# eridgd/WCT-TF

Hardware: AMD Instinct MI355X
Metric: stylized frames/sec @512x512, 5-level relu5->1 pipeline, alpha=0.8 (higher is better)
Workload: dtype f16

## Files before the change

### wct_tf_amd/csrc/conv_wino.hip

```cpp
#include "common.h"

namespace {
typedef unsigned int u32x4 __attribute__((ext_vector_type(4)));
typedef _Float16 h2 __attribute__((ext_vector_type(2)));
constexpr int TW = 16;
constexpr int PITCH = 20;
constexpr int BK = 32;

__device__ __forceinline__ half8 pk_sub(half8 a, half8 b) {
  u32x4 ua = __builtin_bit_cast(u32x4, a), ub = __builtin_bit_cast(u32x4, b), r;
#pragma unroll
  for (int i = 0; i < 4; ++i) {
    unsigned o;
    asm("v_pk_add_f16 %0, %1, %2 neg_lo:[0,1] neg_hi:[0,1]" : "=v"(o) : "v"(ua[i]), "v"(ub[i]));
    r[i] = o;
  }
  return __builtin_bit_cast(half8, r);
}

__device__ __forceinline__ int reflect_idx(int i, int n) {
  if (i < 0) i = -i;
  if (i >= n) i = 2 * n - 2 - i;
  i = i < 0 ? 0 : i;
  return i >= n ? n - 1 : i;
}

template <int TH, int BN, int WM, int WN, bool IL>
__global__ __launch_bounds__(256, TH >= 16 ? 1 : 2)
void conv3x3_wino_kernel(ConvArgs p, int tiles_x, int n_tiles) {
  constexpr int PR = TH / 2;
  constexpr int MT = (PR / 2) / WM;
  constexpr int NT = (BN / 32) / WN;
  constexpr int G = 256 / PR;
  constexpr int SL = (72 + G - 1) / G;
  constexpr int PATCH_BYTES = PR * 4 * PITCH * 64;
  constexpr int DUMP_OFF = 2 * PATCH_BYTES;
  constexpr int PF_TAP = 5;
  static_assert(PR % 2 == 0 && (PR / 2) % WM == 0 && 256 % PR == 0 && WM * WN == 4, "tile shape");

  extern __shared__ __attribute__((aligned(16))) unsigned char smem[];
  const int tid = threadIdx.x, lane = tid & 63, wave = tid >> 6;
  const int wm = wave / WN, wn = wave % WN;
  int bid = blockIdx.x;
  const int ntile = bid % n_tiles;
  bid /= n_tiles;
  const int tx = bid % tiles_x, ty = bid / tiles_x;
  const int b = blockIdx.y;
  const int y0 = ty * TH, x0 = tx * TW, n0 = ntile * BN;

  const int Hin = p.upsample ? p.H / 2 : p.H;
  const int Win = p.upsample ? p.W / 2 : p.W;
  const half_t* xb = p.x + (size_t)b * Hin * Win * p.Cin;
  const __amdgpu_buffer_rsrc_t w_rsrc = __builtin_amdgcn_make_buffer_rsrc((void*)p.w_wino, 0, 0x7FFFFFFF, 0x00020000);
  const __amdgpu_buffer_rsrc_t x_rsrc = __builtin_amdgcn_make_buffer_rsrc((void*)xb, 0, 0x7FFFFFFF, 0x00020000);

  const int lpr = tid / G, ls = tid % G;
  unsigned row_off[4], col_off[SL], dst_off[SL];
  bool slot_ok[SL];
#pragma unroll
  for (int i = 0; i < 4; ++i) {
    int iy = reflect_idx(y0 + 2 * lpr - 1 + i, p.H);
    if (p.upsample) iy >>= 1;
    row_off[i] = (unsigned)(iy * Win) * p.Cin * 2;
  }
#pragma unroll
  for (int j = 0; j < SL; ++j) {
    const int slot = ls + j * G;
    slot_ok[j] = slot < 72;
    const int px = slot_ok[j] ? slot >> 2 : 0, piece = slot & 3;
    int ix = reflect_idx(x0 - 1 + px, p.W);
    if (p.upsample) ix >>= 1;
    col_off[j] = (unsigned)(ix * p.Cin + piece * 8) * 2;
    dst_off[j] = ((lpr * 4 * PITCH + px) * 4 + (piece ^ ((px >> 2) & 3))) * 16;
    if (IL && !slot_ok[j]) dst_off[j] = DUMP_OFF + tid * 16;
  }
  u32x4 raw[SL][4];
  auto load_rows = [&](int chunk) {
#pragma unroll
    for (int j = 0; j < SL; ++j)
#pragma unroll
      for (int i = 0; i < 4; ++i)
        raw[j][i] = __builtin_amdgcn_raw_buffer_load_b128(x_rsrc, row_off[i] + col_off[j], chunk * BK * 2, 0);
  };
  auto park_rows = [&](int buf) {
#pragma unroll
    for (int j = 0; j < SL; ++j) {
      const half8 d0 = __builtin_bit_cast(half8, raw[j][0]), d1 = __builtin_bit_cast(half8, raw[j][1]);
      const half8 d2 = __builtin_bit_cast(half8, raw[j][2]), d3 = __builtin_bit_cast(half8, raw[j][3]);
      const half8 t0 = pk_sub(d0, d2), t1 = d1 + d2, t2 = pk_sub(d2, d1), t3 = pk_sub(d1, d3);
      if (slot_ok[j]) {
        unsigned char* d = smem + buf * PATCH_BYTES + dst_off[j];
        *reinterpret_cast<half8*>(d) = t0;
        *reinterpret_cast<half8*>(d + PITCH * 64) = t1;
        *reinterpret_cast<half8*>(d + 2 * PITCH * 64) = t2;
        *reinterpret_cast<half8*>(d + 3 * PITCH * 64) = t3;
      }
    }
  };

  const int frag_px = lane & 15, frag_pr = (lane & 31) >> 4, kgrp = lane >> 5;
  int rd_base[3][2];
#pragma unroll
  for (int kx = 0; kx < 3; ++kx)
#pragma unroll
    for (int ks = 0; ks < 2; ++ks) {
      const int px = frag_px + kx;
      rd_base[kx][ks] = (((wm * MT * 2 + frag_pr) * 4) * PITCH + px) * 64 + (((ks * 2 + kgrp) ^ ((px >> 2) & 3)) * 16);
    }
  const int c16 = p.Cin >> 4;
  unsigned wfrag[NT];
#pragma unroll
  for (int nt = 0; nt < NT; ++nt) wfrag[nt] = (((n0 >> 5) + wn * NT + nt) * 12 * c16 * 512 + lane * 8) * 2;

  f32x16 acc[4][NT][MT];
#pragma unroll
  for (int nt = 0; nt < NT; ++nt) {
    f32x4 bv[4];
#pragma unroll
    for (int rq = 0; rq < 4; ++rq) bv[rq] = *reinterpret_cast<const f32x4*>(p.bias + n0 + (wn * NT + nt) * 32 + 8 * rq + 4 * kgrp);
#pragma unroll
    for (int f = 0; f < 4; ++f)
#pragma unroll
      for (int mt = 0; mt < MT; ++mt)
#pragma unroll
        for (int r = 0; r < 16; ++r) acc[f][nt][mt][r] = f == 1 ? bv[r >> 2][r & 3] : 0.f;
  }

  const int n_chunks = p.Cin / BK;
  half8 wf[3][NT][2];
  half8 bf[IL ? 3 : 2][2][MT];
  auto load_w = [&](half8 (&dst)[NT][2], int tap12, int chunk) {
    const int soff = (tap12 * c16 + chunk * 2) * 1024;
#pragma unroll
    for (int nt = 0; nt < NT; ++nt)
#pragma unroll
      for (int ks = 0; ks < 2; ++ks)
        dst[nt][ks] = __builtin_bit_cast(half8, __builtin_amdgcn_raw_buffer_load_b128(w_rsrc, wfrag[nt] + ks * 1024, soff, 0));
  };
  auto read_b = [&](half8 (&dst)[2][MT], int f, int kx, int buf) {
#pragma unroll
    for (int ks = 0; ks < 2; ++ks)
#pragma unroll
      for (int mt = 0; mt < MT; ++mt)
        dst[ks][mt] = *reinterpret_cast<const half8*>(smem + buf * PATCH_BYTES + rd_base[kx][ks] + (mt * 8 + f) * PITCH * 64);
  };

  if constexpr (IL) {
    constexpr int NM = 2 * MT * NT;
    constexpr int NR = 2 * NT + 2 * MT;
#ifndef WINO_LT0
#define WINO_LT0 1
#define WINO_PT0 6
#endif
    constexpr int LT0 = WINO_LT0, PT0 = WINO_PT0;
    static_assert(LT0 + SL <= PT0 && PT0 + SL <= 10, "staging schedule");
#ifndef WINO_WRING
#define WINO_WRING 4
#endif
#ifndef WINO_ABL
#define WINO_ABL 0
#endif
#ifndef WINO_RAW_AUX
#define WINO_RAW_AUX 0
#endif
    constexpr int ABL = WINO_ABL;
    constexpr int WR = WINO_WRING, WA = WR - 1;
    static_assert(24 % WR == 0, "ring");
    half8 wq[WR][NT][2];
    half8 tq[4];
    load_rows(0);
#pragma unroll
    for (int i = 0; i < WA; ++i) load_w(wq[i], i, 0);
#pragma unroll
    for (int j = 0; j < SL; ++j) {
      const half8 d0 = __builtin_bit_cast(half8, raw[j][0]), d1 = __builtin_bit_cast(half8, raw[j][1]);
      const half8 d2 = __builtin_bit_cast(half8, raw[j][2]), d3 = __builtin_bit_cast(half8, raw[j][3]);
      unsigned char* d = smem + dst_off[j];
      *reinterpret_cast<half8*>(d) = pk_sub(d0, d2);
      *reinterpret_cast<half8*>(d + PITCH * 64) = d1 + d2;
      *reinterpret_cast<half8*>(d + 2 * PITCH * 64) = pk_sub(d2, d1);
      *reinterpret_cast<half8*>(d + 3 * PITCH * 64) = pk_sub(d1, d3);
    }
    asm volatile("s_waitcnt lgkmcnt(0)\n\ts_barrier" ::: "memory");
    read_b(bf[0], 0, 0, 0);
    read_b(bf[1], 0, 1, 0);
#pragma unroll 1
    for (int pair = 0; pair < n_chunks; pair += 2) {
#pragma unroll
      for (int t = 0; t < 24; ++t) {
        const int tt = t % 12, chunk_i = pair + t / 12, buf = t / 12;
        const int f = tt / 3, kx = tt % 3;
        const int chunk_n = chunk_i + 1 < n_chunks ? chunk_i + 1 : chunk_i;
        const int t3 = (tt + WA) % 12, c3 = tt + WA >= 12 ? chunk_n : chunk_i;
        const int t1 = (tt + 2) % 12, buf1 = tt >= 10 ? buf ^ 1 : buf;
        const int soff3 = (t3 * c16 + c3 * 2) * 1024;
#pragma unroll
        for (int j = 0; j < NM; ++j) {
          const int ks = j / (MT * NT), mt = (j / NT) % MT, nt = j % NT;
          if (!(ABL & 4)) acc[f][nt][mt] = __builtin_amdgcn_mfma_f32_32x32x16_f16(wq[t % WR][nt][ks], bf[t % 3][ks][mt], acc[f][nt][mt], 0, 0, 0);
          else asm volatile("" :: "v"(wq[t % WR][nt][ks]), "v"(bf[t % 3][ks][mt]));
#pragma unroll
          for (int k = j * NR / NM; k < (j + 1) * NR / NM; ++k) {
            if (k < 2 * NT) {
              if (!(ABL & 1)) wq[(t + WA) % WR][k / 2][k % 2] =
                  __builtin_bit_cast(half8, __builtin_amdgcn_raw_buffer_load_b128(w_rsrc, wfrag[k / 2] + (k % 2) * 1024, soff3, 0));
            } else {
              const int kk = k - 2 * NT, ks1 = kk / MT, mt1 = kk % MT;
              if (!(ABL & 8)) bf[(t + 2) % 3][ks1][mt1] = *reinterpret_cast<const half8*>(smem + buf1 * PATCH_BYTES + rd_base[t1 % 3][ks1] + (mt1 * 8 + t1 / 3) * PITCH * 64);
            }
          }
          if (tt >= LT0 && tt < LT0 + SL) {
            const int sl = tt - LT0;
            if (j < 4 && !(ABL & 2)) raw[sl][j] = __builtin_amdgcn_raw_buffer_load_b128(x_rsrc, (ABL & 64) ? (lane & 3) * 16 + j * 64 + sl * 256 : row_off[j] + col_off[sl], (ABL & 32) ? 0 : chunk_n * BK * 2, WINO_RAW_AUX);
          }
          if (tt >= PT0 && tt < PT0 + SL && !(ABL & 16)) {
            const int sl = tt - PT0;
            {
#pragma unroll
              for (int it = j * 8 / NM; it < (j + 1) * 8 / NM; ++it) {
                const int fq = it >> 1;
                if ((it & 1) == 0) {
                  const half8 da = __builtin_bit_cast(half8, raw[sl][fq == 0 ? 0 : fq == 1 ? 1 : fq == 2 ? 2 : 1]);
                  const half8 db = __builtin_bit_cast(half8, raw[sl][fq == 0 ? 2 : fq == 1 ? 2 : fq == 2 ? 1 : 3]);
                  tq[fq] = fq == 1 ? da + db : pk_sub(da, db);
                } else {
                  *reinterpret_cast<half8*>(smem + (buf ^ 1) * PATCH_BYTES * (slot_ok[sl] ? 1 : 0) + dst_off[sl] + fq * PITCH * 64) = tq[fq];
                }
              }
            }
          }
          __builtin_amdgcn_sched_barrier(0);
        }
        if (tt == 9) asm volatile("s_waitcnt lgkmcnt(0)\n\ts_barrier" ::: "memory");
      }
    }
  } else {
  load_rows(0);
  load_w(wf[0], 0, 0);
  load_w(wf[1], 1, 0);
  park_rows(0);
  asm volatile("s_waitcnt lgkmcnt(0)\n\ts_barrier" ::: "memory");
  read_b(bf[0], 0, 0, 0);

#pragma unroll 1
  for (int pair = 0; pair < n_chunks; pair += 2) {
#pragma unroll
    for (int t = 0; t < 24; ++t) {
      const int tt = t % 12, chunk_i = pair + t / 12, buf = t / 12;
      const int f = tt / 3, kx = tt % 3;
      const bool more = chunk_i + 1 < n_chunks;
      {
        const int t2 = (tt + 2) % 12;
        const int c2 = tt + 2 >= 12 ? (more ? chunk_i + 1 : chunk_i) : chunk_i;
        load_w(wf[(t + 2) % 3], t2, c2);
      }
      if (tt == PF_TAP && more) load_rows(chunk_i + 1);
      if (tt != 11) read_b(bf[(t + 1) & 1], (tt + 1) / 3, (tt + 1) % 3, buf);
      else if (more) read_b(bf[(t + 1) & 1], 0, 0, buf ^ 1);
      __builtin_amdgcn_sched_barrier(0);
#pragma unroll
      for (int ks = 0; ks < 2; ++ks)
#pragma unroll
        for (int mt = 0; mt < MT; ++mt)
#pragma unroll
          for (int nt = 0; nt < NT; ++nt)
            acc[f][nt][mt] = __builtin_amdgcn_mfma_f32_32x32x16_f16(wf[t % 3][nt][ks], bf[t & 1][ks][mt], acc[f][nt][mt], 0, 0, 0);
      __builtin_amdgcn_sched_barrier(0);
      if (tt == 10 && more) {
        park_rows(buf ^ 1);
        asm volatile("s_waitcnt lgkmcnt(0)\n\ts_barrier" ::: "memory");
      }
    }
  }

  }
  constexpr int OOB = (int)0x80000000u;
  const int Ho = p.pool ? (p.H + 1) / 2 : p.H, Wo = p.pool ? (p.W + 1) / 2 : p.W;
  const unsigned img_elems = (unsigned)Ho * Wo * p.Cout;
  const __amdgpu_buffer_rsrc_t r16 = __builtin_amdgcn_make_buffer_rsrc((void*)(p.y16 + (size_t)b * img_elems), 0, img_elems * 2, 0x00020000);
  const float lo1 = p.relu ? 0.f : -__builtin_inff();
  const h2 lo2 = {(half_t)lo1, (half_t)lo1};
  const h2 zero2 = {(half_t)0.f, (half_t)0.f};
  const int ox = x0 + frag_px;
  const int chan = n0 + wn * NT * 32;
#pragma unroll
  for (int mt = 0; mt < MT; ++mt) {
    const int oy = y0 + ((wm * MT + mt) * 2 + frag_pr) * 2;
    const bool in0 = (oy < p.H) & (ox < p.W), in1 = (oy + 1 < p.H) & (ox < p.W);
    int off[2];
    if (p.pool) {
      off[0] = in0 && (frag_px & 1) == 0 ? (((oy >> 1) * Wo + (ox >> 1)) * p.Cout + chan + 8 * kgrp) * 2 : OOB;
      off[1] = OOB;
    } else {
      off[0] = in0 ? ((oy * p.W + ox) * p.Cout + chan + 8 * kgrp) * 2 : OOB;
      off[1] = in1 ? (((oy + 1) * p.W + ox) * p.Cout + chan + 8 * kgrp) * 2 : OOB;
    }
#pragma unroll
    for (int nt = 0; nt < NT; ++nt) {
      unsigned pk[2][4][2];
#pragma unroll
      for (int rq = 0; rq < 4; ++rq) {
        f32x4 e, o;
#pragma unroll
        for (int j = 0; j < 4; ++j) {
          const int r = rq * 4 + j;
          const float m0 = acc[0][nt][mt][r], m1 = acc[1][nt][mt][r], m2 = acc[2][nt][mt][r], m3 = acc[3][nt][mt][r];
          e[j] = (m0 + m1) + m2;
          o[j] = (m1 - m2) - m3;
        }
        h2 e0 = {(half_t)e[0], (half_t)e[1]}, e1 = {(half_t)e[2], (half_t)e[3]};
        h2 o0 = {(half_t)o[0], (half_t)o[1]}, o1 = {(half_t)o[2], (half_t)o[3]};
        e0 = __builtin_elementwise_max(e0, lo2); e1 = __builtin_elementwise_max(e1, lo2);
        o0 = __builtin_elementwise_max(o0, lo2); o1 = __builtin_elementwise_max(o1, lo2);
        if (p.pool) {
          h2 q[2] = {__builtin_elementwise_max(in0 ? e0 : zero2, in1 ? o0 : zero2), __builtin_elementwise_max(in0 ? e1 : zero2, in1 ? o1 : zero2)};
#pragma unroll
          for (int d = 0; d < 2; ++d) {
            const unsigned tq = __builtin_bit_cast(unsigned, q[d]);
            const h2 nb = __builtin_bit_cast(h2, __builtin_amdgcn_update_dpp(0, (int)tq, 0xB1, 0xF, 0xF, true));
            q[d] = __builtin_elementwise_max(q[d], nb);
          }
          e0 = q[0]; e1 = q[1];
        }
        pk[0][rq][0] = __builtin_bit_cast(unsigned, e0); pk[0][rq][1] = __builtin_bit_cast(unsigned, e1);
        pk[1][rq][0] = __builtin_bit_cast(unsigned, o0); pk[1][rq][1] = __builtin_bit_cast(unsigned, o1);
      }
#pragma unroll
      for (int par = 0; par < 2; ++par) {
#pragma unroll
        for (int m = 0; m < 2; ++m) {
          auto sx = __builtin_amdgcn_permlane32_swap(pk[par][2 * m][0], pk[par][2 * m + 1][0], false, false);
          auto sy = __builtin_amdgcn_permlane32_swap(pk[par][2 * m][1], pk[par][2 * m + 1][1], false, false);
          u32x4 ov = {sx[0], sy[0], sx[1], sy[1]};
          __builtin_amdgcn_raw_buffer_store_b128(ov, r16, off[par] + (nt * 32 + 16 * m) * 2, 0, 0);
        }
      }
    }
  }
}

template <int TH, int BN, int WM, int WN, bool IL = false>
int launch_wino_cfg(const ConvArgs& a, hipStream_t s) {
  const int tiles_x = cdiv(a.W, TW), tiles_y = cdiv(a.H, TH), n_tiles = a.Cout / BN;
  const size_t lds = 2 * (size_t)(TH / 2) * 4 * PITCH * 64 + (IL ? 8192 : 0);
  HIP_TRY(hipFuncSetAttribute(reinterpret_cast<const void*>(&conv3x3_wino_kernel<TH, BN, WM, WN, IL>),
                              hipFuncAttributeMaxDynamicSharedMemorySize, (int)lds));
  hipLaunchKernelGGL((conv3x3_wino_kernel<TH, BN, WM, WN, IL>), dim3(tiles_x * tiles_y * n_tiles, a.B), dim3(256), lds, s, a, tiles_x, n_tiles);
  HIP_TRY(hipGetLastError());
  return WCT_OK;
}
}

bool conv3x3_wino_takes(const ConvArgs& a) {
  return a.w_wino != nullptr && a.y16 != nullptr && a.y32 == nullptr && a.usum == nullptr && a.img1 == nullptr &&
         a.Cin % 64 == 0 && a.Cout % 64 == 0 && (!a.pool || a.relu);
}

int launch_conv3x3_wino(const ConvArgs& a, hipStream_t s) {
  ARG_CHECK(conv3x3_wino_takes(a) && a.H > 1 && a.W > 1 && a.B > 0);
  ARG_CHECK(!a.upsample || (a.H % 2 == 0 && a.W % 2 == 0));
  ARG_CHECK(launch_map_fits((size_t)a.H * a.W * a.Cin, 2));
  ARG_CHECK(launch_map_fits((size_t)a.H * a.W * a.Cout, 2));
  const long px16 = (long)cdiv(a.W, TW) * cdiv(a.H, 16) * a.B;
  const long px8 = (long)cdiv(a.W, TW) * cdiv(a.H, 8) * a.B;
  if (a.Cout % 128 == 0 && px16 * (a.Cout / 128) >= 256) return launch_wino_cfg<16, 128, 1, 4, true>(a, s);
  if (a.Cout % 128 == 0 && px8 * (a.Cout / 128) >= 256) return launch_wino_cfg<8, 128, 1, 4>(a, s);
  return launch_wino_cfg<8, 64, 2, 2>(a, s);
}
```

Before: 675.5.

## Make the large Winograd conv persistent, prefetching the next tile during the current one

Moves the TH=16 interleaved Winograd path into a new persistent kernel. It launches one block per CU, and each block walks the tiles with a grid stride. During the last chunk pair of a tile it stages the next tile's input rows and weights, so the prologue of each tile overlaps the previous one's compute and the launch/tail cost of many short blocks goes away. Bias is cached in LDS once per block. Risks are extra register pressure from the tile bookkeeping, and lower parallelism if a layer has few tiles or one block per CU underfills the machine.

Measured after the change: 685.3 (median of 6 runs). +1.5%, better.

```diff
diff --git a/wct_tf_amd/csrc/conv_wino.hip b/wct_tf_amd/csrc/conv_wino.hip
--- a/wct_tf_amd/csrc/conv_wino.hip
+++ b/wct_tf_amd/csrc/conv_wino.hip
@@ -25,7 +25,7 @@
   return i >= n ? n - 1 : i;
 }
 
-template <int TH, int BN, int WM, int WN, bool IL>
+template <int TH, int BN, int WM, int WN>
 __global__ __launch_bounds__(256, TH >= 16 ? 1 : 2)
 void conv3x3_wino_kernel(ConvArgs p, int tiles_x, int n_tiles) {
   constexpr int PR = TH / 2;
@@ -34,7 +34,6 @@
   constexpr int G = 256 / PR;
   constexpr int SL = (72 + G - 1) / G;
   constexpr int PATCH_BYTES = PR * 4 * PITCH * 64;
-  constexpr int DUMP_OFF = 2 * PATCH_BYTES;
   constexpr int PF_TAP = 5;
   static_assert(PR % 2 == 0 && (PR / 2) % WM == 0 && 256 % PR == 0 && WM * WN == 4, "tile shape");
 
@@ -72,7 +71,6 @@
     if (p.upsample) ix >>= 1;
     col_off[j] = (unsigned)(ix * p.Cin + piece * 8) * 2;
     dst_off[j] = ((lpr * 4 * PITCH + px) * 4 + (piece ^ ((px >> 2) & 3))) * 16;
-    if (IL && !slot_ok[j]) dst_off[j] = DUMP_OFF + tid * 16;
   }
   u32x4 raw[SL][4];
   auto load_rows = [&](int chunk) {
@@ -128,7 +126,7 @@
 
   const int n_chunks = p.Cin / BK;
   half8 wf[3][NT][2];
-  half8 bf[IL ? 3 : 2][2][MT];
+  half8 bf[2][2][MT];
   auto load_w = [&](half8 (&dst)[NT][2], int tap12, int chunk) {
     const int soff = (tap12 * c16 + chunk * 2) * 1024;
 #pragma unroll
@@ -145,15 +143,252 @@
         dst[ks][mt] = *reinterpret_cast<const half8*>(smem + buf * PATCH_BYTES + rd_base[kx][ks] + (mt * 8 + f) * PITCH * 64);
   };
 
-  if constexpr (IL) {
-    constexpr int NM = 2 * MT * NT;
-    constexpr int NR = 2 * NT + 2 * MT;
+  load_rows(0);
+  load_w(wf[0], 0, 0);
+  load_w(wf[1], 1, 0);
+  park_rows(0);
+  asm volatile("s_waitcnt lgkmcnt(0)\n\ts_barrier" ::: "memory");
+  read_b(bf[0], 0, 0, 0);
+
+#pragma unroll 1
+  for (int pair = 0; pair < n_chunks; pair += 2) {
+#pragma unroll
+    for (int t = 0; t < 24; ++t) {
+      const int tt = t % 12, chunk_i = pair + t / 12, buf = t / 12;
+      const int f = tt / 3, kx = tt % 3;
+      const bool more = chunk_i + 1 < n_chunks;
+      {
+        const int t2 = (tt + 2) % 12;
+        const int c2 = tt + 2 >= 12 ? (more ? chunk_i + 1 : chunk_i) : chunk_i;
+        load_w(wf[(t + 2) % 3], t2, c2);
+      }
+      if (tt == PF_TAP && more) load_rows(chunk_i + 1);
+      if (tt != 11) read_b(bf[(t + 1) & 1], (tt + 1) / 3, (tt + 1) % 3, buf);
+      else if (more) read_b(bf[(t + 1) & 1], 0, 0, buf ^ 1);
+      __builtin_amdgcn_sched_barrier(0);
+#pragma unroll
+      for (int ks = 0; ks < 2; ++ks)
+#pragma unroll
+        for (int mt = 0; mt < MT; ++mt)
+#pragma unroll
+          for (int nt = 0; nt < NT; ++nt)
+            acc[f][nt][mt] = __builtin_amdgcn_mfma_f32_32x32x16_f16(wf[t % 3][nt][ks], bf[t & 1][ks][mt], acc[f][nt][mt], 0, 0, 0);
+      __builtin_amdgcn_sched_barrier(0);
+      if (tt == 10 && more) {
+        park_rows(buf ^ 1);
+        asm volatile("s_waitcnt lgkmcnt(0)\n\ts_barrier" ::: "memory");
+      }
+    }
+  }
+
+  constexpr int OOB = (int)0x80000000u;
+  const int Ho = p.pool ? (p.H + 1) / 2 : p.H, Wo = p.pool ? (p.W + 1) / 2 : p.W;
+  const unsigned img_elems = (unsigned)Ho * Wo * p.Cout;
+  const __amdgpu_buffer_rsrc_t r16 = __builtin_amdgcn_make_buffer_rsrc((void*)(p.y16 + (size_t)b * img_elems), 0, img_elems * 2, 0x00020000);
+  const float lo1 = p.relu ? 0.f : -__builtin_inff();
+  const h2 lo2 = {(half_t)lo1, (half_t)lo1};
+  const h2 zero2 = {(half_t)0.f, (half_t)0.f};
+  const int ox = x0 + frag_px;
+  const int chan = n0 + wn * NT * 32;
+#pragma unroll
+  for (int mt = 0; mt < MT; ++mt) {
+    const int oy = y0 + ((wm * MT + mt) * 2 + frag_pr) * 2;
+    const bool in0 = (oy < p.H) & (ox < p.W), in1 = (oy + 1 < p.H) & (ox < p.W);
+    int off[2];
+    if (p.pool) {
+      off[0] = in0 && (frag_px & 1) == 0 ? (((oy >> 1) * Wo + (ox >> 1)) * p.Cout + chan + 8 * kgrp) * 2 : OOB;
+      off[1] = OOB;
+    } else {
+      off[0] = in0 ? ((oy * p.W + ox) * p.Cout + chan + 8 * kgrp) * 2 : OOB;
+      off[1] = in1 ? (((oy + 1) * p.W + ox) * p.Cout + chan + 8 * kgrp) * 2 : OOB;
+    }
+#pragma unroll
+    for (int nt = 0; nt < NT; ++nt) {
+      unsigned pk[2][4][2];
+#pragma unroll
+      for (int rq = 0; rq < 4; ++rq) {
+        f32x4 e, o;
+#pragma unroll
+        for (int j = 0; j < 4; ++j) {
+          const int r = rq * 4 + j;
+          const float m0 = acc[0][nt][mt][r], m1 = acc[1][nt][mt][r], m2 = acc[2][nt][mt][r], m3 = acc[3][nt][mt][r];
+          e[j] = (m0 + m1) + m2;
+          o[j] = (m1 - m2) - m3;
+        }
+        h2 e0 = {(half_t)e[0], (half_t)e[1]}, e1 = {(half_t)e[2], (half_t)e[3]};
+        h2 o0 = {(half_t)o[0], (half_t)o[1]}, o1 = {(half_t)o[2], (half_t)o[3]};
+        e0 = __builtin_elementwise_max(e0, lo2); e1 = __builtin_elementwise_max(e1, lo2);
+        o0 = __builtin_elementwise_max(o0, lo2); o1 = __builtin_elementwise_max(o1, lo2);
+        if (p.pool) {
+          h2 q[2] = {__builtin_elementwise_max(in0 ? e0 : zero2, in1 ? o0 : zero2), __builtin_elementwise_max(in0 ? e1 : zero2, in1 ? o1 : zero2)};
+#pragma unroll
+          for (int d = 0; d < 2; ++d) {
+            const unsigned tq = __builtin_bit_cast(unsigned, q[d]);
+            const h2 nb = __builtin_bit_cast(h2, __builtin_amdgcn_update_dpp(0, (int)tq, 0xB1, 0xF, 0xF, true));
+            q[d] = __builtin_elementwise_max(q[d], nb);
+          }
+          e0 = q[0]; e1 = q[1];
+        }
+        pk[0][rq][0] = __builtin_bit_cast(unsigned, e0); pk[0][rq][1] = __builtin_bit_cast(unsigned, e1);
+        pk[1][rq][0] = __builtin_bit_cast(unsigned, o0); pk[1][rq][1] = __builtin_bit_cast(unsigned, o1);
+      }
+#pragma unroll
+      for (int par = 0; par < 2; ++par) {
+#pragma unroll
+        for (int m = 0; m < 2; ++m) {
+          auto sx = __builtin_amdgcn_permlane32_swap(pk[par][2 * m][0], pk[par][2 * m + 1][0], false, false);
+          auto sy = __builtin_amdgcn_permlane32_swap(pk[par][2 * m][1], pk[par][2 * m + 1][1], false, false);
+          u32x4 ov = {sx[0], sy[0], sx[1], sy[1]};
+          __builtin_amdgcn_raw_buffer_store_b128(ov, r16, off[par] + (nt * 32 + 16 * m) * 2, 0, 0);
+        }
+      }
+    }
+  }
+}
+
+template <int TH, int BN, int WM, int WN>
+__global__ __launch_bounds__(256, 1)
+void conv3x3_wino_walk_kernel(ConvArgs p, int tiles_x, int n_tiles, int tiles_y, int n_total) {
+  constexpr int PR = TH / 2;
+  constexpr int MT = (PR / 2) / WM;
+  constexpr int NT = (BN / 32) / WN;
+  constexpr int G = 256 / PR;
+  constexpr int SL = (72 + G - 1) / G;
+  constexpr int PATCH_BYTES = PR * 4 * PITCH * 64;
+  constexpr int DUMP_OFF = 2 * PATCH_BYTES;
+  constexpr int BIAS_OFF = DUMP_OFF + 8192;
+  static_assert(PR % 2 == 0 && (PR / 2) % WM == 0 && 256 % PR == 0 && WM * WN == 4, "tile shape");
+
+  extern __shared__ __attribute__((aligned(16))) unsigned char smem[];
+  const int tid = threadIdx.x, lane = tid & 63, wave = tid >> 6;
+  const int wave_s = __builtin_amdgcn_readfirstlane(wave);
+  auto fresh_tid = [&]() {
+    int v;
+    asm volatile("v_mbcnt_lo_u32_b32 %0, -1, 0\n\tv_mbcnt_hi_u32_b32 %0, -1, %0" : "=v"(v));
+    return wave_s * 64 + v;
+  };
+  const int wm = wave / WN, wn = wave % WN;
+  struct Tile { int b, y0, x0, n0; };
+  auto tile_at = [&](int t) {
+    Tile r;
+    r.n0 = (t % n_tiles) * BN;
+    t /= n_tiles;
+    r.x0 = (t % tiles_x) * TW;
+    t /= tiles_x;
+    r.y0 = (t % tiles_y) * TH;
+    r.b = t / tiles_y;
+    return r;
+  };
+  Tile cur = tile_at(blockIdx.x);
+
+  const int Hin = p.upsample ? p.H / 2 : p.H;
+  const int Win = p.upsample ? p.W / 2 : p.W;
+  const __amdgpu_buffer_rsrc_t w_rsrc = __builtin_amdgcn_make_buffer_rsrc((void*)p.w_wino, 0, 0x7FFFFFFF, 0x00020000);
+  auto image_rsrc = [&](int b) { return __builtin_amdgcn_make_buffer_rsrc((void*)(p.x + (size_t)b * Hin * Win * p.Cin), 0, 0x7FFFFFFF, 0x00020000); };
+  __amdgpu_buffer_rsrc_t x_rsrc = image_rsrc(cur.b);
+
+  const int lpr = tid / G, ls = tid % G;
+  unsigned row_off[4], col_off[SL], dst_off[SL];
+  bool slot_ok[SL];
+  auto stage_from = [&](int y0, int x0) {
+    const int tid_s = fresh_tid(), lpr = tid_s / G, ls = tid_s % G;
+#pragma unroll
+    for (int i = 0; i < 4; ++i) {
+      int iy = reflect_idx(y0 + 2 * lpr - 1 + i, p.H);
+      if (p.upsample) iy >>= 1;
+      row_off[i] = (unsigned)(iy * Win) * p.Cin * 2;
+    }
+#pragma unroll
+    for (int j = 0; j < SL; ++j) {
+      const int slot = ls + j * G;
+      const int px = slot < 72 ? slot >> 2 : 0, piece = slot & 3;
+      int ix = reflect_idx(x0 - 1 + px, p.W);
+      if (p.upsample) ix >>= 1;
+      col_off[j] = (unsigned)(ix * p.Cin + piece * 8) * 2;
+    }
+  };
+  stage_from(cur.y0, cur.x0);
+#pragma unroll
+  for (int j = 0; j < SL; ++j) {
+    const int slot = ls + j * G;
+    slot_ok[j] = slot < 72;
+    const int px = slot_ok[j] ? slot >> 2 : 0, piece = slot & 3;
+    dst_off[j] = ((lpr * 4 * PITCH + px) * 4 + (piece ^ ((px >> 2) & 3))) * 16;
+    if (!slot_ok[j]) dst_off[j] = DUMP_OFF + tid * 16;
+  }
+  u32x4 raw[SL][4];
+  auto load_rows = [&](int chunk) {
+#pragma unroll
+    for (int j = 0; j < SL; ++j)
+#pragma unroll
+      for (int i = 0; i < 4; ++i)
+        raw[j][i] = __builtin_amdgcn_raw_buffer_load_b128(x_rsrc, row_off[i] + col_off[j], chunk * BK * 2, 0);
+  };
+
+  const int frag_px = lane & 15, frag_pr = (lane & 31) >> 4, kgrp = lane >> 5;
+  int rd_base[3][2];
+#pragma unroll
+  for (int kx = 0; kx < 3; ++kx)
+#pragma unroll
+    for (int ks = 0; ks < 2; ++ks) {
+      const int px = frag_px + kx;
+      rd_base[kx][ks] = (((wm * MT * 2 + frag_pr) * 4) * PITCH + px) * 64 + (((ks * 2 + kgrp) ^ ((px >> 2) & 3)) * 16);
+    }
+  const int c16 = p.Cin >> 4;
+  unsigned wfrag[NT];
+#pragma unroll
+  for (int nt = 0; nt < NT; ++nt) wfrag[nt] = ((wn * NT + nt) * 12 * c16 * 512 + lane * 8) * 2;
+  auto wtile_off = [&](int n0) { return (unsigned)((n0 >> 5) * 12 * c16 * 1024); };
+
+  f32x16 acc[4][NT][MT];
+  f32x4 bv[NT][4];
+  auto load_bias = [&](int n0) {
+    const int tid_b = fresh_tid(), wn = (tid_b >> 6) % WN, kgrp = (tid_b & 63) >> 5;
+#pragma unroll
+    for (int nt = 0; nt < NT; ++nt)
+#pragma unroll
+      for (int rq = 0; rq < 4; ++rq) {
+        const int c = n0 + (wn * NT + nt) * 32 + 8 * rq + 4 * kgrp;
+        bv[nt][rq] = *reinterpret_cast<const f32x4*>(smem + BIAS_OFF + c * 4);
+      }
+  };
+  auto init_acc = [&]() {
+#pragma unroll
+    for (int nt = 0; nt < NT; ++nt)
+#pragma unroll
+      for (int f = 0; f < 4; ++f)
+#pragma unroll
+        for (int mt = 0; mt < MT; ++mt)
+#pragma unroll
+          for (int r = 0; r < 16; ++r) acc[f][nt][mt][r] = f == 1 ? bv[nt][r >> 2][r & 3] : 0.f;
+  };
+
+  const int n_chunks = p.Cin / BK;
+  half8 bf[3][2][MT];
+  auto load_w = [&](half8 (&dst)[NT][2], int tap12, int chunk, unsigned wt) {
+    const int soff = (tap12 * c16 + chunk * 2) * 1024 + wt;
+#pragma unroll
+    for (int nt = 0; nt < NT; ++nt)
+#pragma unroll
+      for (int ks = 0; ks < 2; ++ks)
+        dst[nt][ks] = __builtin_bit_cast(half8, __builtin_amdgcn_raw_buffer_load_b128(w_rsrc, wfrag[nt] + ks * 1024, soff, 0));
+  };
+  auto read_b = [&](half8 (&dst)[2][MT], int f, int kx, int buf) {
+#pragma unroll
+    for (int ks = 0; ks < 2; ++ks)
+#pragma unroll
+      for (int mt = 0; mt < MT; ++mt)
+        dst[ks][mt] = *reinterpret_cast<const half8*>(smem + buf * PATCH_BYTES + rd_base[kx][ks] + (mt * 8 + f) * PITCH * 64);
+  };
+
+  int tile = blockIdx.x;
+  Tile nxt = cur;
+  unsigned wt_cur = wtile_off(cur.n0), wt_nxt = wt_cur;
+  bool has_next = false;
 #ifndef WINO_LT0
 #define WINO_LT0 1
 #define WINO_PT0 6
 #endif
-    constexpr int LT0 = WINO_LT0, PT0 = WINO_PT0;
-    static_assert(LT0 + SL <= PT0 && PT0 + SL <= 10, "staging schedule");
 #ifndef WINO_WRING
 #define WINO_WRING 4
 #endif
@@ -163,14 +398,15 @@
 #ifndef WINO_RAW_AUX
 #define WINO_RAW_AUX 0
 #endif
-    constexpr int ABL = WINO_ABL;
-    constexpr int WR = WINO_WRING, WA = WR - 1;
-    static_assert(24 % WR == 0, "ring");
-    half8 wq[WR][NT][2];
-    half8 tq[4];
+  constexpr int ABL = WINO_ABL;
+  constexpr int WR = WINO_WRING, WA = WR - 1;
+  static_assert(24 % WR == 0, "ring");
+  half8 wq[WR][NT][2];
+  half8 tq[4];
+  {
     load_rows(0);
 #pragma unroll
-    for (int i = 0; i < WA; ++i) load_w(wq[i], i, 0);
+    for (int i = 0; i < WA; ++i) load_w(wq[i], i, 0, wt_cur);
 #pragma unroll
     for (int j = 0; j < SL; ++j) {
       const half8 d0 = __builtin_bit_cast(half8, raw[j][0]), d1 = __builtin_bit_cast(half8, raw[j][1]);
@@ -181,19 +417,44 @@
       *reinterpret_cast<half8*>(d + 2 * PITCH * 64) = pk_sub(d2, d1);
       *reinterpret_cast<half8*>(d + 3 * PITCH * 64) = pk_sub(d1, d3);
     }
+    for (int c = tid * 4; c < p.Cout; c += 1024) *reinterpret_cast<f32x4*>(smem + BIAS_OFF + c * 4) = *reinterpret_cast<const f32x4*>(p.bias + c);
     asm volatile("s_waitcnt lgkmcnt(0)\n\ts_barrier" ::: "memory");
+  }
+#pragma unroll 1
+  for (;;) {
+  {
+    constexpr int NM = 2 * MT * NT;
+    constexpr int NR = 2 * NT + 2 * MT;
+    constexpr int LT0 = WINO_LT0, PT0 = WINO_PT0;
+    static_assert(LT0 + SL <= PT0 && PT0 + SL <= 10, "staging schedule");
+    has_next = tile + (int)gridDim.x < n_total;
     read_b(bf[0], 0, 0, 0);
     read_b(bf[1], 0, 1, 0);
+    load_bias(cur.n0);
+    init_acc();
 #pragma unroll 1
-    for (int pair = 0; pair < n_chunks; pair += 2) {
+    for (int pair = 0;;) {
+      int stage_c = pair + 2;
+      unsigned stage_wt = wt_cur;
 #pragma unroll
       for (int t = 0; t < 24; ++t) {
         const int tt = t % 12, chunk_i = pair + t / 12, buf = t / 12;
         const int f = tt / 3, kx = tt % 3;
-        const int chunk_n = chunk_i + 1 < n_chunks ? chunk_i + 1 : chunk_i;
+        if (t == 12 && pair + 2 >= n_chunks) {
+          stage_c = pair + 1;
+          if (has_next) {
+            nxt = tile_at(tile + (int)gridDim.x);
+            stage_c = 0;
+            stage_wt = wt_nxt = wtile_off(nxt.n0);
+            stage_from(nxt.y0, nxt.x0);
+            x_rsrc = image_rsrc(nxt.b);
+          }
+        }
+        const int chunk_n = t < 12 ? pair + 1 : stage_c;
+        const unsigned wt_n = t < 12 ? wt_cur : stage_wt;
         const int t3 = (tt + WA) % 12, c3 = tt + WA >= 12 ? chunk_n : chunk_i;
         const int t1 = (tt + 2) % 12, buf1 = tt >= 10 ? buf ^ 1 : buf;
-        const int soff3 = (t3 * c16 + c3 * 2) * 1024;
+        const int soff3 = (t3 * c16 + c3 * 2) * 1024 + (tt + WA >= 12 ? wt_n : wt_cur);
 #pragma unroll
         for (int j = 0; j < NM; ++j) {
           const int ks = j / (MT * NT), mt = (j / NT) % MT, nt = j % NT;
@@ -233,59 +494,26 @@
         }
         if (tt == 9) asm volatile("s_waitcnt lgkmcnt(0)\n\ts_barrier" ::: "memory");
       }
-    }
-  } else {
-  load_rows(0);
-  load_w(wf[0], 0, 0);
-  load_w(wf[1], 1, 0);
-  park_rows(0);
-  asm volatile("s_waitcnt lgkmcnt(0)\n\ts_barrier" ::: "memory");
-  read_b(bf[0], 0, 0, 0);
-
-#pragma unroll 1
-  for (int pair = 0; pair < n_chunks; pair += 2) {
-#pragma unroll
-    for (int t = 0; t < 24; ++t) {
-      const int tt = t % 12, chunk_i = pair + t / 12, buf = t / 12;
-      const int f = tt / 3, kx = tt % 3;
-      const bool more = chunk_i + 1 < n_chunks;
-      {
-        const int t2 = (tt + 2) % 12;
-        const int c2 = tt + 2 >= 12 ? (more ? chunk_i + 1 : chunk_i) : chunk_i;
-        load_w(wf[(t + 2) % 3], t2, c2);
-      }
-      if (tt == PF_TAP && more) load_rows(chunk_i + 1);
-      if (tt != 11) read_b(bf[(t + 1) & 1], (tt + 1) / 3, (tt + 1) % 3, buf);
-      else if (more) read_b(bf[(t + 1) & 1], 0, 0, buf ^ 1);
-      __builtin_amdgcn_sched_barrier(0);
-#pragma unroll
-      for (int ks = 0; ks < 2; ++ks)
-#pragma unroll
-        for (int mt = 0; mt < MT; ++mt)
-#pragma unroll
-          for (int nt = 0; nt < NT; ++nt)
-            acc[f][nt][mt] = __builtin_amdgcn_mfma_f32_32x32x16_f16(wf[t % 3][nt][ks], bf[t & 1][ks][mt], acc[f][nt][mt], 0, 0, 0);
-      __builtin_amdgcn_sched_barrier(0);
-      if (tt == 10 && more) {
-        park_rows(buf ^ 1);
-        asm volatile("s_waitcnt lgkmcnt(0)\n\ts_barrier" ::: "memory");
-      }
-    }
-  }
-
-  }
+      if ((pair += 2) >= n_chunks) break;
+    }
+  }
+  const int tid_e = fresh_tid();
+  const int lane_e = tid_e & 63, wn = (tid_e >> 6) % WN, wm = (tid_e >> 6) / WN;
+  const int frag_px = lane_e & 15, frag_pr = (lane_e & 31) >> 4, kgrp = lane_e >> 5;
   constexpr int OOB = (int)0x80000000u;
   const int Ho = p.pool ? (p.H + 1) / 2 : p.H, Wo = p.pool ? (p.W + 1) / 2 : p.W;
   const unsigned img_elems = (unsigned)Ho * Wo * p.Cout;
-  const __amdgpu_buffer_rsrc_t r16 = __builtin_amdgcn_make_buffer_rsrc((void*)(p.y16 + (size_t)b * img_elems), 0, img_elems * 2, 0x00020000);
-  const float lo1 = p.relu ? 0.f : -__builtin_inff();
+  const __amdgpu_buffer_rsrc_t r16 = __builtin_amdgcn_make_buffer_rsrc((void*)(p.y16 + (size_t)cur.b * img_elems), 0, img_elems * 2, 0x00020000);
+  int relu = p.relu;
+  asm volatile("" : "+s"(relu));
+  const float lo1 = relu ? 0.f : -__builtin_inff();
   const h2 lo2 = {(half_t)lo1, (half_t)lo1};
   const h2 zero2 = {(half_t)0.f, (half_t)0.f};
-  const int ox = x0 + frag_px;
-  const int chan = n0 + wn * NT * 32;
+  const int ox = cur.x0 + frag_px;
+  const int chan = cur.n0 + wn * NT * 32;
 #pragma unroll
   for (int mt = 0; mt < MT; ++mt) {
-    const int oy = y0 + ((wm * MT + mt) * 2 + frag_pr) * 2;
+    const int oy = cur.y0 + ((wm * MT + mt) * 2 + frag_pr) * 2;
     const bool in0 = (oy < p.H) & (ox < p.W), in1 = (oy + 1 < p.H) & (ox < p.W);
     int off[2];
     if (p.pool) {
@@ -337,15 +565,37 @@
       }
     }
   }
-}
-
-template <int TH, int BN, int WM, int WN, bool IL = false>
+  if (!has_next) break;
+  tile += gridDim.x;
+  cur = nxt;
+  wt_cur = wt_nxt;
+  }
+}
+
+template <int TH, int BN, int WM, int WN>
 int launch_wino_cfg(const ConvArgs& a, hipStream_t s) {
   const int tiles_x = cdiv(a.W, TW), tiles_y = cdiv(a.H, TH), n_tiles = a.Cout / BN;
-  const size_t lds = 2 * (size_t)(TH / 2) * 4 * PITCH * 64 + (IL ? 8192 : 0);
-  HIP_TRY(hipFuncSetAttribute(reinterpret_cast<const void*>(&conv3x3_wino_kernel<TH, BN, WM, WN, IL>),
+  const size_t lds = 2 * (size_t)(TH / 2) * 4 * PITCH * 64;
+  HIP_TRY(hipFuncSetAttribute(reinterpret_cast<const void*>(&conv3x3_wino_kernel<TH, BN, WM, WN>),
                               hipFuncAttributeMaxDynamicSharedMemorySize, (int)lds));
-  hipLaunchKernelGGL((conv3x3_wino_kernel<TH, BN, WM, WN, IL>), dim3(tiles_x * tiles_y * n_tiles, a.B), dim3(256), lds, s, a, tiles_x, n_tiles);
+  hipLaunchKernelGGL((conv3x3_wino_kernel<TH, BN, WM, WN>), dim3(tiles_x * tiles_y * n_tiles, a.B), dim3(256), lds, s, a, tiles_x, n_tiles);
+  HIP_TRY(hipGetLastError());
+  return WCT_OK;
+}
+
+template <int TH, int BN, int WM, int WN>
+int launch_wino_walk(const ConvArgs& a, hipStream_t s) {
+  const int tiles_x = cdiv(a.W, TW), tiles_y = cdiv(a.H, TH), n_tiles = a.Cout / BN;
+  const long total = (long)tiles_x * tiles_y * n_tiles * a.B;
+  const size_t lds = 2 * (size_t)(TH / 2) * 4 * PITCH * 64 + 8192 + 4 * (size_t)a.Cout;
+  int dev = 0, cus = 0;
+  HIP_TRY(hipGetDevice(&dev));
+  HIP_TRY(hipDeviceGetAttribute(&cus, hipDeviceAttributeMultiprocessorCount, dev));
+  ARG_CHECK(cus > 0 && total < (1L << 30) && lds <= 160 * 1024);
+  HIP_TRY(hipFuncSetAttribute(reinterpret_cast<const void*>(&conv3x3_wino_walk_kernel<TH, BN, WM, WN>),
+                              hipFuncAttributeMaxDynamicSharedMemorySize, (int)lds));
+  hipLaunchKernelGGL((conv3x3_wino_walk_kernel<TH, BN, WM, WN>), dim3((unsigned)(total < cus ? total : cus)), dim3(256), lds, s, a, tiles_x,
+                     n_tiles, tiles_y, (int)total);
   HIP_TRY(hipGetLastError());
   return WCT_OK;
 }
@@ -363,7 +613,7 @@
   ARG_CHECK(launch_map_fits((size_t)a.H * a.W * a.Cout, 2));
   const long px16 = (long)cdiv(a.W, TW) * cdiv(a.H, 16) * a.B;
   const long px8 = (long)cdiv(a.W, TW) * cdiv(a.H, 8) * a.B;
-  if (a.Cout % 128 == 0 && px16 * (a.Cout / 128) >= 256) return launch_wino_cfg<16, 128, 1, 4, true>(a, s);
+  if (a.Cout % 128 == 0 && px16 * (a.Cout / 128) >= 256) return launch_wino_walk<16, 128, 1, 4>(a, s);
   if (a.Cout % 128 == 0 && px8 * (a.Cout / 128) >= 256) return launch_wino_cfg<8, 128, 1, 4>(a, s);
   return launch_wino_cfg<8, 64, 2, 2>(a, s);
 }
```
